# resero-labs/latok

Measured on AMD Instinct MI355X. Metric: input UTF-8 GB/s tokenized (fused feature+split-mask path), higher is better.
Workload: dtype u64

## Files before the change

### latok_amd/csrc/api.cpp

```cpp
#include <hip/hip_runtime.h>
#include <errno.h>
#include <fcntl.h>
#include <stdarg.h>
#include <stdio.h>
#include <stdlib.h>
#include <string.h>
#include <sys/mman.h>
#include <sys/stat.h>
#include <unistd.h>

#include <algorithm>
#include <array>
#include <atomic>
#include <chrono>
#include <mutex>
#include <new>
#include <string>
#include <thread>
#include <vector>

#include "../../include/latok_hip.h"
#include "corpus_gen.h"
#include "flow_hazards.h"
#include "kernels.h"
#include "unicode_tables.inc"

static_assert(LATOK_TBL_SHIFT == latok::kTblShift, "table shift");
static_assert(LATOK_TBL_STAGE1_LEN == latok::kStage1Len, "stage-1 length");
static_assert(LATOK_TBL_NBLOCKS * (1 << LATOK_TBL_SHIFT) == latok::kStage2Len, "stage-2 length");
static_assert(LATOK_TILE_CHARS == latok::kTile, "tile size");

namespace {

thread_local std::string g_err;

int fail(int code, const char* fmt, ...) {
    char buf[512];
    va_list ap;
    va_start(ap, fmt);
    vsnprintf(buf, sizeof(buf), fmt, ap);
    va_end(ap);
    g_err = buf;
    return code;
}
#define HIP_TRY(expr)                                                                                     \
    do {                                                                                                  \
        hipError_t e_ = (expr);                                                                           \
        if (e_ != hipSuccess) return fail(LATOK_ERR_HIP, "%s failed: %s", #expr, hipGetErrorString(e_)); \
    } while (0)

struct DevBuf {
    void* p = nullptr;
    size_t cap = 0;
    unsigned gen = 0;
    int ensure(size_t bytes) {
        if (bytes <= cap) return LATOK_OK;
        ++gen;
        if (p) (void)hipFree(p);
        p = nullptr;
        cap = 0;
        size_t want = bytes + bytes / 8 + 256;
        hipError_t e = hipMalloc(&p, want);
        if (e != hipSuccess) {
            p = nullptr;
            return fail(LATOK_ERR_NOMEM, "hipMalloc(%zu) failed: %s", want, hipGetErrorString(e));
        }
        cap = want;
        return LATOK_OK;
    }
    void release() {
        if (p) (void)hipFree(p);
        p = nullptr;
        cap = 0;
    }
};

struct PinBuf {
// ... 263 lines not shown
    P.u8 = in.form == Form::Utf32 ? nullptr : (const uint8_t*)in.p;
    P.row_off = a.b.row;
    P.n_str = n_str;
    P.total = total;
    P.n_tiles = n_tiles;
    const int n_cu = g.plan_cus > 0 ? g.plan_cus : g.n_cu;
    const bool one_launch_ok = a.stages == 7 && in.form == Form::Utf32 && !a.tiles_begin && !a.tiles_end && one_segment_enabled();
    latok::LaunchPlan L;
    latok::plan_launch(n_tiles, n_cu, &w != &g.ws, mode, one_launch_ok, &L);
    P.seg_tiles = L.seg_tiles;
    P.n_segs = L.n_segs;
    const bool one_launch = L.one_launch != 0;
    if ((size_t)P.n_segs * (sizeof(latok::Fn64) + sizeof(latok::Hd64)) > w.seg_agg.cap || (size_t)n_tiles * 16 > w.summ.cap)
        return fail(LATOK_ERR_INVALID, "internal: workspace too small for %lld segments / %lld tiles", (long long)P.n_segs, (long long)n_tiles);
    if (a.codes && mode != latok::kModeBits && mode != latok::kModeRules)
        return fail(LATOK_ERR_INVALID, "internal: code bytes are written by the UTF-32 bitmask modes only");
    const uint8_t* tables = (const uint8_t*)((latok::mode_rules(mode) || a.codes) ? g.t1rule.p : g.t1.p);
    P.t1 = tables;
    P.t2 = tables + latok::kStage1Pad;
    if (latok::mode_base(mode) == latok::kModeBytes) {
        P.t1 = (const uint8_t*)(latok::mode_rules(mode) ? g.tb6rule.p : g.tb6.p);
        P.t2 = P.t1 + latok::kB6Stage1Bytes;
    }
    if (latok::mode_rules(mode)) P.rules = g.rules;
    else memset(&P.rules, 0, sizeof(P.rules));
    P.bits_out = a.bits;
    P.values_out = a.values;
    P.space_out = a.space;
    P.lead_out = a.lead;
    P.lead_pref_out = a.lead_pref;
    P.lead_cnt_out = a.lead_cnt;
    P.codes_out = a.codes;
    P.tile_first = (int64_t*)w.tile_first.p;
    P.summ = (int4*)w.summ.p;
    P.seg_fn = (latok::Fn64*)w.seg_agg.p;
    P.seg_hd = (latok::Hd64*)((char*)w.seg_agg.p + (size_t)P.n_segs * sizeof(latok::Fn64));
    P.fix_count = (int64_t*)w.fix_count.p;
    P.bm_a1 = a.bm_a1;
    P.bm_a2 = a.bm_a2;
    P.bm_flags = a.bm_flags;
    P.done = (a.stages & 4) ? a.done : latok::DoneSignal{nullptr, 0, nullptr};
    g.last.plan = L;
    g.last.n_tiles = n_tiles;
    g.last.mode = mode;
    g.last.small = g.pin.d && in.p == g.pin.d;
    g.last.fix_count = (const int64_t*)w.fix_count.p;
    g.last.st = a.st;
    g.last.valid = true;
    const hipStream_t st = a.st;
    if (one_launch) {
        HIP_TRY(latok::launch_one_segment(P, mode, st));
        return LATOK_OK;
    }
    if (a.stages & 1) HIP_TRY(latok::launch_tile_index(P, st));
    if (a.tiles_begin) HIP_TRY(hipEventRecord(a.tiles_begin, st));
    if (a.stages & 2) HIP_TRY(latok::launch_split_tiles(P, mode, L, st));
    if (a.tiles_end) HIP_TRY(hipEventRecord(a.tiles_end, st));
    if (a.stages & 4) HIP_TRY(latok::launch_resolve_fix(P, mode, L, st));
    return LATOK_OK;
}

int check_csr_host(const int64_t* row_off, int64_t n_str, int64_t* total_io) {
    if (n_str < 0) return fail(LATOK_ERR_INVALID, "n_str must be >= 0");
    if (n_str == 0) { *total_io = 0; return LATOK_OK; }
    if (!row_off) return fail(LATOK_ERR_INVALID, "row_off is NULL");
    if (row_off[0] != 0) return fail(LATOK_ERR_INVALID, "row_off[0] must be 0");
    for (int64_t s = 0; s < n_str; ++s)
        if (row_off[s + 1] < row_off[s]) return fail(LATOK_ERR_INVALID, "row_off must be non-decreasing");
    if (*total_io >= 0 && *total_io != row_off[n_str])
        return fail(LATOK_ERR_INVALID, "total_chars does not match row_off[n_str]");
    *total_io = row_off[n_str];
    return LATOK_OK;
}

int resolve_total_device(const int64_t* d_row, int64_t n_str, int64_t* total_io, hipStream_t st) {
    if (n_str < 0) return fail(LATOK_ERR_INVALID, "n_str must be >= 0");
    if (n_str == 0) { *total_io = 0; return LATOK_OK; }
    if (*total_io < 0) {
        HIP_TRY(hipMemcpyAsync(total_io, d_row + n_str, 8, hipMemcpyDeviceToHost, st));
        HIP_TRY(hipStreamSynchronize(st));
    }
    return LATOK_OK;
}

int resolve_total(const int64_t* row_off, int64_t n_str, int64_t* total_io, bool dev, hipStream_t st) {
    return dev ? resolve_total_device(row_off, n_str, total_io, st) : check_csr_host(row_off, n_str, total_io);
}

int arm_done(Ctx& g, hipStream_t st, latok::DoneSignal* done) {
    *done = latok::DoneSignal{nullptr, 0, nullptr};
    if (!poll_completion()) return LATOK_OK;
    int rc;
    if ((rc = g.pin_tot.ensure(64)) || (rc = g.done_ctr.ensure(64))) return rc;
    if (g.done_ctr.gen != g.done_ctr_seen) {
        g.done_ctr_seen = g.done_ctr.gen;
        HIP_TRY(hipMemsetAsync(g.done_ctr.p, 0, 64, st));
    }
    *done = latok::DoneSignal{(unsigned long long*)g.pin_tot.d + 2, ++g.small_seq, (unsigned*)g.done_ctr.p};
    return LATOK_OK;
}
int wait_done(Ctx& g, const latok::DoneSignal& done, hipStream_t st) {
    if (!(done.word && wait_completion_word((const unsigned long long*)g.pin_tot.h + 2, done.seq))) HIP_TRY(hipStreamSynchronize(st));
    return LATOK_OK;
}

int units_on_device(Ctx& g, const Batch& b, bool dev, hipStream_t st, Batch* d) {
    *d = b;
// ... 1768 lines not shown
}
int latok_utf8_bytes(const uint32_t* cps, int64_t n, int64_t* bytes_out, int flags) {
    if (!bytes_out || n < 0) return fail(LATOK_ERR_INVALID, "bad args");
    if (!(flags & LATOK_DEVICE_PTRS)) {
        int64_t t = 0;
        for (int64_t i = 0; i < n; ++i) t += latok_utf8_len(cps[i]);
        *bytes_out = t;
        return LATOK_OK;
    }
    LATOK_ENTER();
    int rc = need_init(g);
    if (rc) return rc;
    HIP_TRY(latok::launch_utf8_bytes(cps, n, (unsigned long long*)g.ws.scalar.p, g.stream));
    unsigned long long t = 0;
    HIP_TRY(hipMemcpyAsync(&t, g.ws.scalar.p, 8, hipMemcpyDeviceToHost, g.stream));
    HIP_TRY(hipStreamSynchronize(g.stream));
    *bytes_out = (int64_t)t;
    return LATOK_OK;
}

int latok_debug_set_scan_epoch(unsigned epoch) {
    LATOK_ENTER();
    g.ws.scan_epoch = epoch & 0x3FFFFu;
    return LATOK_OK;
}

extern "C" int latok_debug_limits(int64_t* out, int n) {
    const int64_t v[17] = {latok::kTile, latok::kWPB, latok::kNarrowWPB, latok::kSegMax, latok::kOneSegTiles, latok::kFastTailTiles,
                           kSmallChars, kSmallStrings, latok::kCompressWaves, latok::kFeatWaves, latok::kFeatRound, latok::kFeatRoundTm,
                           latok::kFeatFormThresh, latok::kFeatWinBytes, latok::kHashWaveBytes, latok::scan_small_max(),
                           latok::utf8_block_bytes()};
    if (!out || n < 0) return fail(LATOK_ERR_INVALID, "NULL output");
    const int k = n < 17 ? n : 17;
    for (int i = 0; i < k; ++i) out[i] = v[i];
    return k;
}

static int put_plan(const latok::LaunchPlan& L, int64_t n_tiles, int64_t* out, int n) {
    const int64_t v[12] = {L.n_cu_eff, L.seg_tiles, L.n_segs, L.rounds, L.grid, L.one_launch ? 0 : L.grid, L.fast_tail, L.pf, L.wpb, L.nw,
                           L.one_launch, n_tiles};
    const int k = n < 12 ? n : 12;
    for (int i = 0; i < k; ++i) out[i] = v[i];
    return k;
}

extern "C" int latok_debug_plan(int64_t n_tiles, int n_cu, int in_flow, int mode, int64_t* out, int n) {
    if (!out || n < 0 || n_tiles < 1 || n_cu < 1 || mode < latok::kModeBits || mode > latok::kModeValuesRules)
        return fail(LATOK_ERR_INVALID, "n_tiles >= 1, n_cu >= 1, mode 0..%d", latok::kModeValuesRules);
    latok::LaunchPlan L;
    latok::plan_launch(n_tiles, n_cu, in_flow != 0, mode, one_segment_enabled(), &L);
    return put_plan(L, n_tiles, out, n);
}

extern "C" int latok_debug_set_plan_cus(int n_cu) {
    LATOK_ENTER();
    int rc = need_init(g);
    if (rc) return rc;
    if (n_cu != 0 && (n_cu < 8 || n_cu > g.n_cu)) return fail(LATOK_ERR_INVALID, "plan CUs must be 0 or 8..%d", g.n_cu);
    g.plan_cus = n_cu;
    return LATOK_OK;
}

extern "C" int latok_debug_last_plan(int64_t* out, int n) {
    LATOK_ENTER();
    int rc = need_init(g);
    if (rc) return rc;
    if (!out || n < 0) return fail(LATOK_ERR_INVALID, "NULL output");
    if (!g.last.valid) return 0;
    int64_t fix = 0;
    HIP_TRY(hipStreamSynchronize(g.last.st));
    HIP_TRY(hipMemcpy(&fix, g.last.fix_count, 8, hipMemcpyDeviceToHost));
    const int64_t head[3] = {g.last.mode, g.last.small ? 1 : 0, fix};
    int k = 0;
    for (; k < 3 && k < n; ++k) out[k] = head[k];
    if (n > 3) k += put_plan(g.last.plan, g.last.n_tiles, out + 3, n - 3);
    return k;
}

extern "C" int latok_debug_last_route(void) {
    LATOK_ENTER();
    return g.last_route;
}

extern "C" int latok_debug_flow_route(int n_slots, const uint64_t* lo, const uint64_t* bytes, const int* is_write, int n, int* drained_out) {
    static thread_local latok::FlowHazards held;
    static thread_local unsigned long long seq = 0;
    if (drained_out) *drained_out = 0;
    if (n < 0) { held.clear(); seq = 0; return 0; }
    if (n_slots < 1 || n_slots > latok::FlowHazards::kMaxSlots || n > 16) return fail(LATOK_ERR_INVALID, "1..4 slots, <= 16 ranges");
    latok::FlowRange r[16];
    for (int i = 0; i < n; ++i) r[i] = latok::flow_range((const void*)(uintptr_t)lo[i], (size_t)bytes[i], is_write[i] != 0);
    const int turn = (int)(seq % (unsigned)n_slots);
    int s = held.route(n_slots, turn, r, n);
    if (s == latok::FlowHazards::kDrainFirst) {
        held.clear();
        if (drained_out) *drained_out = 1;
        s = turn;
    }
    held.note(s, r, n);
    ++seq;
    return s;
}

extern "C" int latok_debug_host_decode_utf8(const uint8_t* utf8, const int64_t* byte_off, int64_t n_str, uint32_t* cps_out,
                                            int64_t* cp_row_out, int64_t* bytepos_out, int64_t* n_cps_out) {
    int64_t total = -1;
// ... 910 lines not shown
```

### latok_amd/csrc/aux_kernels.hip

```cpp
#include <hip/hip_runtime.h>
#include <stdint.h>

#include "corpus_gen.h"
#include "kernels.h"
#include "utf8_decode.h"
#include "wave_ops.h"

namespace latok {

__device__ __forceinline__ uint32_t base_word(const uint8_t* t1, const uint8_t* t2cls, const uint16_t* cw, uint32_t cp) {
    const uint32_t hi = min(cp >> kTblShift, (uint32_t)(kStage1Len - 1));
    return cw[t2cls[((uint32_t)t1[hi] << kTblShift) | (cp & ((1u << kTblShift) - 1u))]];
}

__device__ __forceinline__ uint32_t feature_row_bits(uint32_t w, uint32_t p, uint32_t x, uint32_t y, bool first, bool last) {
    uint32_t r = w & 0xFFFu;
    r |= ((p >> 0) & 1u) << 12;
    r |= ((x >> 0) & 1u) << 13;
    r |= ((p >> 1) & 1u) << 14;
    r |= ((x >> 1) & 1u) << 15;
    r |= ((p >> 3) & 1u) << 16;
    r |= ((x >> 3) & 1u) << 17;
    r |= (first ? 1u : (p >> 5) & 1u) << 18;
    r |= (last ? 1u : (x >> 5) & 1u) << 19;
    r |= ((p >> 6) & 1u) << 20;
    r |= ((x >> 8) & 1u) << 21;
    r |= ((x >> 10) & 1u) << 22;
    r |= ((y >> 0) & 1u) << 23;
    r |= ((y >> 10) & 1u) << 24;
    return r;
}

__global__ void k_parse_matrix(const uint32_t* __restrict__ cps, int64_t n, const uint8_t* __restrict__ t1,
                               const uint8_t* __restrict__ t2cls, const uint16_t* __restrict__ cw,
                               int8_t* __restrict__ out) {
    const int64_t i = (int64_t)blockIdx.x * blockDim.x + threadIdx.x;
    if (i >= n) return;
    const uint32_t w = base_word(t1, t2cls, cw, cps[i]);
    const uint32_t p = i > 0 ? base_word(t1, t2cls, cw, cps[i - 1]) : 0u;
    const uint32_t x = i + 1 < n ? base_word(t1, t2cls, cw, cps[i + 1]) : 0u;
    const uint32_t y = i + 2 < n ? base_word(t1, t2cls, cw, cps[i + 2]) : 0u;
    const uint32_t bits = feature_row_bits(w, p, x, y, i == 0, i + 1 == n);
    int8_t* row = out + i * 25;
#pragma unroll
    for (int c = 0; c < 25; ++c) row[c] = (int8_t)((bits >> c) & 1u);
}

hipError_t launch_parse_matrix(const uint32_t* cps, int64_t n, const uint8_t* t1, const uint8_t* t2cls,
                               const uint16_t* cw, int8_t* out, hipStream_t st) {
    if (n <= 0) return hipSuccess;
    const int threads = 256;
    hipLaunchKernelGGL(k_parse_matrix, dim3((unsigned)((n + threads - 1) / threads)), dim3(threads), 0, st, cps, n, t1,
                       t2cls, cw, out);
    return hipGetLastError();
}

__global__ __launch_bounds__(256) void k_parse_matrix_small(const uint32_t* __restrict__ cps, int n, const uint8_t* __restrict__ t1,
// ... 356 lines not shown
hipError_t launch_utf8_decode(const uint8_t* u8, int64_t total, const int64_t* byte_off, int64_t n_str,
                              const int64_t* block_base, uint16_t* chunk_pref, int64_t total_cps, uint32_t* cps,
                              int64_t* cp_off, hipStream_t st) {
    hipLaunchKernelGGL(k_utf8_decode_chunks, dim3((unsigned)utf8_blocks(total)), dim3(kU8Threads), 0, st, u8, total,
                       block_base, chunk_pref, cps);
    hipLaunchKernelGGL(k_utf8_cp_offsets, dim3((unsigned)((n_str + 1 + 255) / 256)), dim3(256), 0, st, u8, total, byte_off,
                       n_str, block_base, chunk_pref, total_cps, cp_off);
    return hipGetLastError();
}

template <typename T>
__global__ void k_widen_units(const T* __restrict__ units, int64_t n, uint32_t* __restrict__ cps) {
    const int64_t i0 = ((int64_t)blockIdx.x * blockDim.x + threadIdx.x) * 4;
    if (i0 + 4 <= n && ((uintptr_t)units & (4 * sizeof(T) - 1)) == 0) {
        T u[4];
        if (sizeof(T) == 1) *reinterpret_cast<uint32_t*>(u) = *reinterpret_cast<const uint32_t*>(units + i0);
        else *reinterpret_cast<uint2*>(u) = *reinterpret_cast<const uint2*>(units + i0);
        *reinterpret_cast<uint4*>(cps + i0) = make_uint4(u[0], u[1], u[2], u[3]);
    } else {
        for (int64_t i = i0; i < n && i < i0 + 4; ++i) cps[i] = units[i];
    }
}

hipError_t launch_widen_units(const void* units, int kind, int64_t n, uint32_t* cps, hipStream_t st) {
    if (n <= 0) return hipSuccess;
    const unsigned blocks = (unsigned)((n + 1023) / 1024);
    if (kind == 1) hipLaunchKernelGGL(k_widen_units<uint8_t>, dim3(blocks), dim3(256), 0, st, (const uint8_t*)units, n, cps);
    else hipLaunchKernelGGL(k_widen_units<uint16_t>, dim3(blocks), dim3(256), 0, st, (const uint16_t*)units, n, cps);
    return hipGetLastError();
}

__global__ void k_corpus_fill(uint64_t seed, int model, uint64_t sid0, int64_t n_str,
                              const int64_t* __restrict__ row_off, uint32_t* __restrict__ cps) {
    const int64_t s = (int64_t)blockIdx.x * blockDim.x + threadIdx.x;
    if (s >= n_str) return;
    const int64_t b = row_off[s];
    latok_corpus_string(seed, model, sid0 + (uint64_t)s, cps + b, row_off[s + 1] - b);
}

hipError_t launch_corpus_fill(uint64_t seed, int model, uint64_t sid0, int64_t n_str, const int64_t* row_off,
                              uint32_t* cps, hipStream_t st) {
    if (n_str <= 0) return hipSuccess;
    hipLaunchKernelGGL(k_corpus_fill, dim3((unsigned)((n_str + 63) / 64)), dim3(64), 0, st, seed, model, sid0, n_str,
                       row_off, cps);
    return hipGetLastError();
}

typedef uint32_t stream_u32x4 __attribute__((ext_vector_type(4)));
__global__ void __launch_bounds__(512) k_stream_read(const stream_u32x4* __restrict__ src, int64_t n_steps,
                                                     uint32_t* __restrict__ sink) {
    const int lane = threadIdx.x & 63;
    const int64_t wave = ((int64_t)blockIdx.x * blockDim.x + threadIdx.x) >> 6;
    const int64_t n_waves = ((int64_t)gridDim.x * blockDim.x) >> 6;
    uint32_t acc = 0;
    for (int64_t t = wave; t < n_steps; t += n_waves) {
        const stream_u32x4* p = src + t * 1024 + lane;
        stream_u32x4 v[16];
#pragma unroll
        for (int i = 0; i < 16; ++i) v[i] = __builtin_nontemporal_load(p + 64 * i);
#pragma unroll
        for (int i = 0; i < 16; ++i) acc ^= v[i].x ^ v[i].y ^ v[i].z ^ v[i].w;
    }
    if (acc == 0x9E3779B9u) sink[0] = acc;
}

hipError_t launch_stream_read(const void* src, int64_t bytes, uint32_t* sink, int n_cu, hipStream_t st) {
    const int64_t n_steps = bytes / 16384;
    if (n_steps <= 0) return hipSuccess;
    hipLaunchKernelGGL(k_stream_read, dim3((unsigned)(n_cu * 2)), dim3(512), 0, st, (const stream_u32x4*)src, n_steps, sink);
    return hipGetLastError();
}

__global__ void k_utf8_bytes(const uint32_t* __restrict__ cps, int64_t n, unsigned long long* __restrict__ total) {
    long long local = 0;
    for (int64_t i = (int64_t)blockIdx.x * blockDim.x + threadIdx.x; i < n; i += (int64_t)gridDim.x * blockDim.x)
        local += latok_utf8_len(cps[i]);
#pragma unroll
    for (int d = 32; d >= 1; d >>= 1) local += __shfl_xor(local, d);
    if ((threadIdx.x & 63) == 0) atomicAdd(total, (unsigned long long)local);
}

hipError_t launch_utf8_bytes(const uint32_t* cps, int64_t n, unsigned long long* total, hipStream_t st) {
    hipError_t e = hipMemsetAsync(total, 0, sizeof(unsigned long long), st);
    if (e != hipSuccess || n <= 0) return e;
    int64_t blocks = (n + 255) / 256;
    if (blocks > 4096) blocks = 4096;
    hipLaunchKernelGGL(k_utf8_bytes, dim3((unsigned)blocks), dim3(256), 0, st, cps, n, total);
    return hipGetLastError();
}

}
```

### latok_amd/csrc/kernels.h

```cpp
#ifndef LATOK_KERNELS_H
#define LATOK_KERNELS_H
#include <hip/hip_runtime.h>
#include <stdint.h>

#include "split_code.h"

namespace latok {

constexpr int kTile = 4096;
constexpr int kTblShift = 7;
constexpr int kStage1Len = 8705;
constexpr int kStage1Pad = 8720;
constexpr int kStage2Len = 255 * 128;
constexpr int kTablesLdsBytes = kStage1Pad + kStage2Len;
constexpr int kB6Stage1Len = LK_B6_STAGE1_LEN;
constexpr int kB6Stage1Bytes = (kB6Stage1Len * 2 + 1023) / 1024 * 1024;
constexpr int kB6MaxBlocks = 400;
constexpr int kB6Stage2Bytes = kB6MaxBlocks * 64;
constexpr int kB6TablesBytes = kB6Stage1Bytes + kB6Stage2Bytes;
static_assert(kB6Stage1Bytes % 1024 == 0 && kB6Stage2Bytes % 1024 == 0 && kB6Stage1Bytes <= kTablesLdsBytes, "byte space keeps its stage 1 where the other modes keep both stages");
constexpr int kStageBytes = 64 * 80;
constexpr int kWaveLdsBytes = kStageBytes + 16 + 65 * 8 + 8;

constexpr int kModeBits = 0;
constexpr int kModeValues = 1;
constexpr int kModeBlockMask = 2;
constexpr int kModeRules = 3;
constexpr int kModeBytes = 4;
constexpr int kModeLatin1 = 5;
constexpr int kModeUcs2 = 6;
constexpr int kModeBytesRules = 7;
constexpr int kModeLatin1Rules = 8;
constexpr int kModeUcs2Rules = 9;
constexpr int kModeValuesRules = 10;
constexpr int mode_base(int mode) {
    return mode == kModeRules ? kModeBits : mode == kModeBytesRules ? kModeBytes : mode == kModeLatin1Rules ? kModeLatin1
         : mode == kModeUcs2Rules ? kModeUcs2 : mode == kModeValuesRules ? kModeValues : mode;
}
constexpr bool mode_rules(int mode) { return mode != mode_base(mode); }
constexpr int mode_with_rules(int base) {
    return base == kModeBits ? kModeRules : base == kModeBytes ? kModeBytesRules : base == kModeLatin1 ? kModeLatin1Rules
         : base == kModeUcs2 ? kModeUcs2Rules : base == kModeValues ? kModeValuesRules : base;
}
constexpr bool mode_is_bytes(int mode) { return mode_base(mode) == kModeBytes || mode_base(mode) == kModeLatin1 || mode_base(mode) == kModeUcs2; }
constexpr bool mode_is_units(int mode) { return mode_base(mode) == kModeLatin1 || mode_base(mode) == kModeUcs2; }
constexpr bool mode_writes_bits(int mode) { return mode_base(mode) == kModeBits || mode_is_bytes(mode); }

constexpr long long kNegInf64 = -(1ll << 60);
constexpr int kWPB = 12;
constexpr int kSegMax = kWPB * 64;

struct Fn64 {
    long long a, b;
};
struct Hd64 {
    long long h;
    int c;
};

struct DoneSignal {
    unsigned long long* word;
    unsigned long long seq;
    unsigned* counter;
};
#if defined(__HIPCC__)
__device__ __forceinline__ void signal_block_done(const DoneSignal& d) {
    if (!d.word) return;
    __threadfence_system();
    __syncthreads();
    if (threadIdx.x == 0) {
        const unsigned n = gridDim.x;
        if (__hip_atomic_fetch_add(d.counter, 1u, __ATOMIC_ACQ_REL, __HIP_MEMORY_SCOPE_AGENT) == n - 1u) {
            *d.counter = 0u;
            __threadfence_system();
            __hip_atomic_store(d.word, d.seq, __ATOMIC_RELEASE, __HIP_MEMORY_SCOPE_SYSTEM);
        }
    }
}
#endif

struct SplitParams {
    const uint32_t* cps;
    const uint8_t* u8;
    const int64_t* row_off;
    int64_t n_str, total, n_tiles;
    int seg_tiles;
    int64_t n_segs;
    const uint8_t* t1;
    const uint8_t* t2;
    uint64_t* bits_out;
    uint8_t* values_out;
    uint64_t* space_out;
    uint64_t* lead_out;
    uint16_t* lead_pref_out;
    int64_t* lead_cnt_out;
    uint8_t* codes_out;
    int64_t* tile_first;
    int4* summ;
    Fn64* seg_fn;
// ... 139 lines not shown
```

### latok_amd/csrc/split_kernels.hip

```cpp
#include <hip/hip_runtime.h>
#include <stdint.h>
#include <stdlib.h>

#include "bitscan.h"
#include "feat_records.h"
#include "kernels.h"
#include "tile_core.h"

namespace latok {

#ifdef LATOK_STAMPS
__device__ unsigned long long g_stamp_sum[16];
__device__ unsigned long long g_stamp_cnt;
#endif

__device__ __forceinline__ Fn64 fn_then(Fn64 f1, Fn64 f2) {
    Fn64 f;
    const bool c1 = f1.a <= kNegInf64, c2 = f2.a <= kNegInf64;
    if (c2) { f.a = kNegInf64; f.b = f2.b; return f; }
    f.a = c1 ? kNegInf64 : f1.a + f2.a;
    const long long c = f1.b + f2.a;
    f.b = c > f2.b ? c : f2.b;
    return f;
}
__device__ __forceinline__ long long fn_apply(Fn64 f, long long q) {
    if (f.a <= kNegInf64) return f.b;
    const long long c = q + f.a;
    return c > f.b ? c : f.b;
}
__device__ __forceinline__ Fn64 fn_of(int4 s) {
    Fn64 f;
    f.a = s.x <= LK_NEG_INF / 2 ? kNegInf64 : (long long)s.x;
    f.b = s.y;
    return f;
}
__device__ __forceinline__ Hd64 hd_then(Hd64 x, Hd64 y) {
    Hd64 r;
    r.c = x.c | y.c;
    r.h = x.c ? x.h : x.h + y.h;
    return r;
}

constexpr int kScanWaves = kWPB;

__device__ __forceinline__ Fn64 fn_identity() { Fn64 f; f.a = 0; f.b = 0; return f; }
__device__ __forceinline__ Hd64 hd_identity() { Hd64 h; h.h = 0; h.c = 0; return h; }

template <int NW>
struct ScanLdsT {
    Fn64 fn_w[NW];
    Hd64 hd_w[NW];
};
typedef ScanLdsT<kScanWaves> ScanLds;
template <int NW = kScanWaves>
__device__ __forceinline__ void block_scan(Fn64 f, Hd64 h, ScanLdsT<NW>& L, Fn64* excl_fn, Hd64* excl_hd, Fn64* tot_fn,
                                           Hd64* tot_hd) {
    const int lane = threadIdx.x & 63, wave = threadIdx.x >> 6;
    Fn64 fi = f;
    Hd64 hi = h;
#pragma unroll
// ... 147 lines not shown
    }
}
__device__ __attribute__((noinline, cold)) void tables_fetch_bytes(const uint8_t* t1, const uint8_t* t2, uint8_t* tables, int* ctl) {
    const int lane = (int)(threadIdx.x & 63u);
    struct { const uint8_t* t1; const uint8_t* t2; } P = {t1, t2};
    struct { uint8_t* tables; int* ctl; } L = {tables, ctl};
    typedef const void __attribute__((address_space(1))) * gptr_t;
    typedef void __attribute__((address_space(3))) * lptr_t;
    for (;;) {
        const int ticket = __hip_atomic_fetch_add(&L.ctl[0], 1, __ATOMIC_RELAXED, __HIP_MEMORY_SCOPE_WORKGROUP);
        const int g = __builtin_amdgcn_readfirstlane(ticket) >> 6;
        if (g >= kLazyGrabs) break;
        if (g == kLazyGrabs - 1) {
#pragma unroll
            for (int j = 0; j < 4; ++j) {
                const lk_lead_entry e = lk_lead_entry_of((uint32_t)(64 * j + lane));
                reinterpret_cast<uint2*>(L.tables + kLdsLeadTab)[64 * j + lane] = make_uint2(e.sel, e.hi0);
            }
        } else {
#pragma unroll
            for (int j = 0; j < kLazyPer; ++j) {
                const int row = g * kLazyPer + j;
                if (row < kLazyRows)
                    __builtin_amdgcn_global_load_lds((gptr_t)(P.t1 + 1024 * row + 16 * lane), (lptr_t)(L.tables + 1024 * row), 16, 0, 0);
            }
            __builtin_amdgcn_s_waitcnt(0x0F70);
        }
        __hip_atomic_fetch_add(&L.ctl[1], 1, __ATOMIC_RELEASE, __HIP_MEMORY_SCOPE_WORKGROUP);
    }
    while (__hip_atomic_load(&L.ctl[1], __ATOMIC_ACQUIRE, __HIP_MEMORY_SCOPE_WORKGROUP) < 64 * kLazyGrabs) __builtin_amdgcn_s_sleep(2);
}

template <int MODE = kModeBits>
__device__ __forceinline__ TileLds wave_lds(uint8_t* lds, int wave) {
    TileLds L;
    L.t1 = lds;
    L.t2 = lds + kStage1Pad;
    uint8_t* const w = lds + lds_shift(MODE);
    uint8_t* mine = wave < kWPB ? w + kLdsWaves + wave * kWaveLdsBytes : lds + lds_total(MODE) + (wave - kWPB) * kWaveLdsBytes;
    L.stage = mine;
    L.halo = mine + kStageBytes;
    L.bw = reinterpret_cast<lk_u64*>(mine + kStageBytes + 16);
    L.lut = lds;
    L.ltab = lds + kLdsLeadTab;
    L.tables = lds;
    L.ctl = reinterpret_cast<int*>(w + kLdsMisc) + 16;
    L.t1b = lds;
    L.t2b = lds + kB6Stage1Bytes;
    L.ctab = mode_base(MODE) == kModeBytes ? lds + kLdsByteCodes : L.lut + kSliceLutBytes;
    L.small_bits = L.small_space = nullptr;
    return L;
}

template <int MODE, bool FAST_TAIL = false, int WPB = kWPB, int PF = kCpsPrefetchRows>
__device__ __forceinline__ void run_segment(const SplitParams& P, uint8_t* lds, int64_t seg, int tid, int lane,
                                            int wave, bool tables LATOK_STAMP_PARAM) {
    const int S = P.seg_tiles;
    const TileLds L = wave_lds<MODE>(lds, wave);
    int4* sm = reinterpret_cast<int4*>(lds + lds_shift(MODE) + kLdsSumm);
    ScanLdsT<WPB>& scan = *reinterpret_cast<ScanLdsT<WPB>*>(lds + lds_shift(MODE) + kLdsScan);

    const int64_t T0 = seg * S;
    const int64_t T1 = min(T0 + S, P.n_tiles);
    const int n_seg = (int)(T1 - T0);
    int64_t tfv = 0;
    if (wave + WPB * lane < n_seg) tfv = P.tile_first[T0 + wave + WPB * lane];
    tfv = tfv < 0 ? 0 : (tfv > P.n_str ? P.n_str : tfv);
    if (tables) __syncthreads();
    constexpr bool kDefer = mode_writes_bits(MODE) && !mode_is_bytes(MODE);
    lk_u64 obuf[8];
    int slot = 0, k_first = wave;
    const int64_t n_words = (P.total + 63) >> 6;
    auto flush = [&]() {
#pragma unroll
        for (int j = 0; j < 8; ++j) {
            if (j < slot) {
                const int64_t w = (T0 + k_first + j * WPB) * 64 + lane;
                if (w < n_words) P.bits_out[w] = obuf[j];
            }
        }
        slot = 0;
    };
    auto put = [&](lk_u64 w, int k) {
        if (slot == 0) k_first = k;
#pragma unroll
        for (int j = 0; j < 8; ++j) obuf[j] = (j == slot) ? w : obuf[j];
        if (++slot == 8) flush();
    };
    CpsPrefetch pf;
    pf.valid = false;
    for (int k = wave, j = 0; k < n_seg; k += WPB, ++j) {
        const lk_u64 w = process_tile<MODE, kDefer, false, FAST_TAIL, PF>(P, L, T0 + k, lane_read64(tfv, j), 0, -1, true, &sm[k], lane LATOK_STAMP_ARG
                                                                      , MODE == kModeBits && !FAST_TAIL ? &pf : nullptr, k + WPB < n_seg ? T0 + k + WPB : (int64_t)-1
                                                                      );
        if (kDefer) put(w, k);
#ifdef LATOK_STAMPS
        stamp_acc[0] += 1;
#endif
    }
    if (kDefer) flush();
    __syncthreads();
    {
        Fn64 f = fn_identity();
        Hd64 h = hd_identity();
        if (tid < n_seg) {
            const int4 s = sm[tid];
            P.summ[T0 + tid] = s;
            f = fn_of(s);
            h.h = s.z; h.c = s.w & 1;
        }
        Fn64 ef, tfn; Hd64 eh, th;
        block_scan<WPB>(f, h, scan, &ef, &eh, &tfn, &th);
        if (tid == 0) { P.seg_fn[seg] = tfn; P.seg_hd[seg] = th; }
    }
    __syncthreads();
}

template <int MODE, bool FAST_TAIL = false, int PF = kCpsPrefetchRows>
__global__ __launch_bounds__(tile_wpb(MODE) * 64) void k_tiles_main(SplitParams P) {
    constexpr int WPB = tile_wpb(MODE);
    __shared__ __attribute__((aligned(16))) uint8_t lds[lds_total_tiles(MODE)];
    const int tid = threadIdx.x;
    const int lane = tid & 63;
    const int wave = __builtin_amdgcn_readfirstlane(tid >> 6);
    if (blockIdx.x == 0 && tid == 0) *P.fix_count = 0;

    bool tables = MODE != kModeBlockMask;
    if (tables) {
        if (mode_base(MODE) == kModeBytes) load_tables_ascii_bytes(lds, P);
        else load_tables<WPB * 64, MODE>(lds, P);
    }
#ifdef LATOK_STAMPS
    unsigned long long stamp_acc[16];
    for (int i = 0; i < 16; ++i) stamp_acc[i] = 0;
#endif
    for (int64_t seg = blockIdx.x; seg < P.n_segs; seg += gridDim.x) {
        run_segment<MODE, FAST_TAIL, WPB, PF>(P, lds, seg, tid, lane, wave, tables LATOK_STAMP_ARG);
        tables = false;
    }
#ifdef LATOK_STAMPS
    if (lane == 0)
        for (int i = 0; i < 16; ++i) atomicAdd(&g_stamp_sum[i], stamp_acc[i]);
#endif
}

template <int MODE, int NW, bool ONE>
__device__ __forceinline__ void resolve_segments(const SplitParams& P, uint8_t* lds, int tid, int lane, int wave) {
    const int S = P.seg_tiles;
    ScanLdsT<NW>& scan = *reinterpret_cast<ScanLdsT<NW>*>(lds + lds_shift(MODE) + kLdsScan);
    int* misc = reinterpret_cast<int*>(lds + lds_shift(MODE) + kLdsMisc);
    int* fix_t = reinterpret_cast<int*>(lds + lds_shift(MODE) + kLdsTf);
    int2* fix_in = reinterpret_cast<int2*>(lds + lds_shift(MODE) + kLdsSumm);
    bool tables_loaded = ONE;

    for (int64_t seg = ONE ? 0 : (int64_t)blockIdx.x; seg < (ONE ? 1 : P.n_segs); seg += ONE ? 1 : (int64_t)gridDim.x) {
        const int64_t T0 = seg * S;
        const int64_t T1 = min(T0 + S, P.n_tiles);
        const int n_seg = (int)(T1 - T0);
        if (tid == 0) misc[0] = 0;
        const int64_t t = T0 + tid;
        int4 s = make_int4(0, 0, 0, 0);
        if (tid < n_seg) s = P.summ[t];
        Fn64 pf = fn_identity();
        Hd64 sh = hd_identity();
        if (P.n_segs > 1) {
            const int64_t per = (P.n_segs + NW * 64 - 1) / (NW * 64);
            const int64_t lo = min((int64_t)tid * per, P.n_segs), hi = min(lo + per, P.n_segs);
            Fn64 f = fn_identity();
            Hd64 h = hd_identity();
            for (int64_t j = lo; j < hi; ++j) {
                if (j < seg) f = fn_then(f, P.seg_fn[j]);
                if (j > seg) h = hd_then(h, P.seg_hd[j]);
            }
            Fn64 ef; Hd64 eh;
            block_scan<NW>(f, h, scan, &ef, &eh, &pf, &sh);
        }
        const long long q_seg_in = fn_apply(pf, 0);
        Hd64 rest; rest.h = sh.h; rest.c = 1;

        Fn64 f = fn_identity();
        Hd64 h = hd_identity();
        if (tid < n_seg) {
            f = fn_of(s);
            h.h = s.z; h.c = s.w & 1;
        }
        Fn64 ef, tfn; Hd64 eh, th;
        block_scan<NW>(f, h, scan, &ef, &eh, &tfn, &th);
        if (tid < n_seg) {
            const long long q_in = fn_apply(ef, q_seg_in);
            const long long q_end = fn_apply(f, q_in);
            const long long h_next = hd_then(eh, rest).h;
// ... 46 lines not shown
                process_tile<MODE>(P, L, tt, idx0, in.x, in.y, false, nullptr, lane);
            }
            if (tid == 0) atomicAdd(reinterpret_cast<unsigned long long*>(P.fix_count), (unsigned long long)n_fix);
        }
        __syncthreads();
    }
}

template <int MODE, int NW>
__global__ __launch_bounds__(NW * 64) void k_resolve_fix(SplitParams P) {
    __shared__ __attribute__((aligned(16))) uint8_t lds[lds_total(MODE)];
    const int tid = threadIdx.x;
    const int lane = tid & 63;
    const int wave = __builtin_amdgcn_readfirstlane(tid >> 6);
    resolve_segments<MODE, NW, false>(P, lds, tid, lane, wave);
    signal_block_done(P.done);
}

__device__ __forceinline__ void tile_index_entry(const int64_t* __restrict__ row_off, int64_t n_str, int64_t n_tiles,
                                                 int64_t* __restrict__ tile_first, int64_t s, int lane) {
    int64_t w0 = 0, w1 = -1;
    if (s <= n_str) {
        const int64_t p = row_off[s];
        const int64_t prev = s > 0 ? row_off[s - 1] : -1;
        w0 = prev < 0 ? 0 : prev / kTile + 1;
        w1 = p / kTile;
        if (w1 > n_tiles - 1) w1 = n_tiles - 1;
    }
    const bool wide = w1 - w0 >= 16;
    if (!wide)
        for (int64_t w = w0; w <= w1; ++w) tile_first[w] = s;
    unsigned long long m = __ballot(wide);
    while (m) {
        const int src = __ffsll((long long)m) - 1;
        m &= m - 1;
        const int64_t a = lane_read64(w0, src), b = lane_read64(w1, src), v = lane_read64(s, src);
        for (int64_t w = a + lane; w <= b; w += 64) tile_first[w] = v;
    }
}


template <int MODE>
__global__ __launch_bounds__(kWPB * 64) void k_one_segment(SplitParams P) {
    __shared__ __attribute__((aligned(16))) uint8_t lds[lds_total(MODE)];
    const int tid = threadIdx.x;
    const int lane = tid & 63;
    const int wave = __builtin_amdgcn_readfirstlane(tid >> 6);
    if (tid == 0) *P.fix_count = 0;
    load_tables<kWPB * 64, MODE>(lds, P);
    for (int64_t base = 0; base <= P.n_str; base += kWPB * 64)
        tile_index_entry(P.row_off, P.n_str, P.n_tiles, P.tile_first, base + tid, lane);
    __threadfence_block();
    __syncthreads();
    run_segment<MODE, true>(P, lds, 0, tid, lane, wave, true LATOK_STAMP_NULL);
    __threadfence_block();
    __syncthreads();
    resolve_segments<MODE, kWPB, true>(P, lds, tid, lane, wave);
    signal_block_done(P.done);
}

__global__ void k_any_nonzero(const int8_t* __restrict__ a1, const int8_t* __restrict__ a2, int64_t n,
                              int* __restrict__ flags) {
    int f1 = 0, f2 = 0;
    for (int64_t i = (int64_t)blockIdx.x * blockDim.x + threadIdx.x; i < n; i += (int64_t)gridDim.x * blockDim.x) {
        f1 |= a1[i] != 0;
        f2 |= a2[i] != 0;
    }
    if (__any(f1) && (threadIdx.x & 63) == 0) atomicOr(&flags[0], 1);
    if (__any(f2) && (threadIdx.x & 63) == 0) atomicOr(&flags[1], 1);
}

hipError_t launch_any_nonzero(const int8_t* a1, const int8_t* a2, int64_t n, int* flags, hipStream_t st) {
    hipError_t e = hipMemsetAsync(flags, 0, 2 * sizeof(int), st);
    if (e != hipSuccess || n <= 0) return e;
    int64_t blocks = (n + 255) / 256;
    if (blocks > 1024) blocks = 1024;
    hipLaunchKernelGGL(k_any_nonzero, dim3((unsigned)blocks), dim3(256), 0, st, a1, a2, n, flags);
    return hipGetLastError();
}

struct SmallParams {
    SplitParams P;
    void* counts;
    void* items;
    int64_t* n_items;
    unsigned long long* done;
    unsigned long long seq;
    int8_t* features;
};

template <int MODE, int KIND, typename OUT>
__global__ __launch_bounds__(64) void k_small_batch(SmallParams S) {
    __shared__ __attribute__((aligned(16))) uint8_t lds[kWaveLdsBytes];
    __shared__ uint64_t s_bits[66], s_space[66], s_items[66];
    __shared__ int s_pref[66];
    const int lane = threadIdx.x;
    TileLds L;
    L.t1 = S.P.t1;
    L.t2 = S.P.t2;
    L.lut = L.ctab = L.ltab = L.t1b = L.t2b = nullptr; L.tables = nullptr; L.ctl = nullptr;
    L.stage = lds;
    L.halo = lds + kStageBytes;
    L.bw = reinterpret_cast<lk_u64*>(lds + kStageBytes + 16);
    s_bits[lane] = 0ull;
    s_space[lane] = ~0ull;
    if (lane < 2) { s_bits[64 + lane] = 0ull; s_space[64 + lane] = ~0ull; }
    const SplitParams& P = S.P;
// ... 337 lines not shown
```

### latok_amd/csrc/tile_core.h

```cpp
#ifndef LATOK_TILE_CORE_H
#define LATOK_TILE_CORE_H
#include <hip/hip_runtime.h>
#include <stdint.h>

#include "kernels.h"
#include "lane_math.h"
#include "utf8_decode.h"
#include "wave_ops.h"

namespace latok {

#ifdef LATOK_STAMPS
#define LATOK_STAMP(k)                                                                           \
    do {                                                                                         \
        __builtin_amdgcn_sched_barrier(0);                                                       \
        unsigned long long t_;                                                                   \
        asm volatile("s_memtime %0\n\ts_waitcnt lgkmcnt(0)" : "=s"(t_)::"memory");            \
        __builtin_amdgcn_sched_barrier(0);                                                       \
        if ((k) > 0) stamp_acc[(k)] += t_ - stamp_prev;                                          \
        stamp_prev = t_;                                                                         \
    } while (0)
#define LATOK_STAMP_ARG , stamp_acc
#define LATOK_STAMP_PARAM , unsigned long long* stamp_acc
#define LATOK_STAMP_NULL , nullptr
// ... 681 lines not shown
                            for (int c = 0; c < LK_COUNT_BITS; ++c) {
                                v |= (int)((counts.split[c] >> i) & 1) << c;
                                vy |= (int)((counts.sym[c] >> i) & 1) << c;
                            }
                        } else {
                            v = (int)((loc.t_space >> i) & 1) + (int)((loc.t_sym >> i) & 1) + (int)((loc.t_prevsym >> i) & 1) +
                                (int)((loc.t_camel_next >> i) & 1) + (int)((loc.t_camel_prev >> i) & 1);
                            vy = (int)((loc.sym >> i) & 1);
                        }
                        v = ((keep >> i) & 1) ? v : 0;
                        v += vy;
                        if ((B >> i) & 1) v = 1;
                        packed |= (uint32_t)v << (8 * b);
                    }
                }
                if (4 * w + 4 <= n) {
                    *reinterpret_cast<uint32_t*>(dst + 4 * w) = packed;
                } else {
                    for (int b = 0; b < 4 && 4 * w + b < n; ++b) dst[4 * w + b] = (uint8_t)(packed >> (8 * b));
                }
            }
        }
    }
    if (mode_base(MODE) == kModeBytes && !SMALL && P.lead_out) {
        const int64_t remain = total - base;
        const lk_u64 valid = remain >= 64 ? ~0ull : (remain <= 0 ? 0ull : ((1ull << remain) - 1ull));
        const lk_u64 leadw = ~cont_plane & valid;
        const int cnt = lk_popc(leadw);
        int inc = cnt;
        inc += dpp_mov<kDppRowShr1, 0xF>(0, inc);
        inc += dpp_mov<kDppRowShr2, 0xF>(0, inc);
        inc += dpp_mov<kDppRowShr4, 0xF>(0, inc);
        inc += dpp_mov<kDppRowShr8, 0xF>(0, inc);
        inc += dpp_mov<kDppRowBcast15, 0xA>(0, inc);
        inc += dpp_mov<kDppRowBcast31, 0xC>(0, inc);
        if (base < total) {
            P.lead_out[base >> 6] = leadw;
            P.lead_pref_out[base >> 6] = (uint16_t)(inc - cnt);
        }
        if (lane == 63) P.lead_cnt_out[t] = inc;
    }
    LATOK_STAMP(8);
    wave_lds_sync();
    return out_word;
}


template <int MODE, bool DEFER = false, bool SMALL = false, bool FAST_TAIL = false, int PF = kCpsPrefetchRows>
__device__ __forceinline__ lk_u64 process_tile(const SplitParams& P, const TileLds& L, int64_t t, int64_t idx0, int q_in,
                                             int tail_zero, bool write_summary, int4* summ_l, int lane
#ifdef LATOK_STAMPS
                                             , unsigned long long* stamp_acc = nullptr
#endif
                                             , CpsPrefetch* pf = nullptr, int64_t t_next = -1
                                             ) {
#ifdef LATOK_STAMPS
    unsigned long long stamp_prev = 0, stamp_dummy[16];
    if (!stamp_acc) stamp_acc = stamp_dummy;
#endif
    const int64_t t0 = t * kTile;
    const int64_t total = P.total;
    const uint32_t st_lane = 4u * lane + 16u * ((uint32_t)lane >> 4);
    bool raw_stage = mode_base(MODE) == kModeLatin1;
    bool ascii_tile = false;
    bool tile_not_ascii = false;
    LATOK_STAMP(0);

    int64_t ro = idx0 + lane <= P.n_str ? P.row_off[idx0 + lane] : INT64_MAX;
    uint32_t halo_cp = 0xFFFFFFFFu;
    if (MODE != kModeBlockMask && !mode_is_bytes(MODE) && lane < 3) {
        const int64_t hp = lane == 0 ? t0 - 1 : t0 + kTile + (lane - 1);
        if (hp >= 0 && hp < total) halo_cp = P.cps[hp];
    }

    if (MODE == kModeBlockMask) {
    } else if (mode_base(MODE) == kModeLatin1) {
        ascii_tile = units_phase1<1>(P, L, t0, lane);
    } else if (mode_base(MODE) == kModeUcs2) {
        units_phase1<2>(P, L, t0, lane);
    } else if (mode_base(MODE) == kModeBytes) {
        raw_stage = bytes_phase1(P, L, t0, lane
#ifdef LATOK_STAMPS
                                 , stamp_acc, stamp_prev
#endif
                                 );
        ascii_tile = raw_stage;
    } else if (FAST_TAIL) {
        const bool full = t0 + kTile <= total;
        u32x4 v[16];
        const u32x4* src = reinterpret_cast<const u32x4*>(P.cps + t0) + lane;
        const int64_t remain0 = total - t0 - 4 * (int64_t)lane;
        int n_rows = 16;
        if (full) {
#pragma unroll
            for (int i = 0; i < 16; ++i) v[i] = __builtin_nontemporal_load(src + 64 * i);
        } else {
            const int64_t last_blk = (total - 1) & ~(int64_t)3;
            n_rows = (int)((total - t0 + 255) >> 8);
#pragma unroll
            for (int i = 0; i < 16; ++i) {
                if (i < n_rows) {
                    int64_t p = t0 + 256 * i + 4 * (int64_t)lane;
                    p = p < last_blk ? p : last_blk;
                    v[i] = __builtin_nontemporal_load(reinterpret_cast<const u32x4*>(P.cps + p));
                }
            }
        }
        uint32_t* codes = P.codes_out ? reinterpret_cast<uint32_t*>(P.codes_out + t0) + lane : nullptr;
#pragma unroll
        for (int i = 0; i < 16; ++i) {
            uint32_t c = 0;
            if (i < n_rows) {
                c = classify4(L.t1, L.t2, v[i]);
                if (!full) {
                    const int64_t remain = remain0 - 256 * i;
                    c &= remain >= 4 ? 0xFFFFFFFFu : (remain <= 0 ? 0u : ((1u << (8 * (int)remain)) - 1u));
                }
            }
            *reinterpret_cast<uint32_t*>(L.stage + st_lane + 320u * i) = c;
            if (codes) codes[64 * i] = c;
        }
    } else if (t0 + kTile <= total) {
        u32x4 v[16];
        const u32x4* src = reinterpret_cast<const u32x4*>(P.cps + t0) + lane;
        constexpr int R = PF;
        const bool pre = R > 0 && pf && pf->valid;
#pragma unroll
        for (int i = 0; i < 16; ++i) {
            if (i < R && pre) v[i] = pf->v[i < R ? i : 0];
            else v[i] = __builtin_nontemporal_load(src + 64 * i);
        }
        LATOK_STAMP(1);
        uint32_t* codes = P.codes_out ? reinterpret_cast<uint32_t*>(P.codes_out + t0) + lane : nullptr;
#pragma unroll
        for (int i = 0; i < 16; ++i) {
            const uint32_t c = classify4(L.t1, L.t2, v[i], &tile_not_ascii);
            *reinterpret_cast<uint32_t*>(L.stage + st_lane + 320u * i) = c;
            if (codes) codes[64 * i] = c;
        }
    } else {
        uint32_t* codes = P.codes_out ? reinterpret_cast<uint32_t*>(P.codes_out + t0) + lane : nullptr;
#pragma unroll 1
        for (int i = 0; i < 16; ++i) {
            const int64_t p = t0 + 256 * i + 4 * lane;
            u32x4 v;
            v.x = p + 0 < total ? P.cps[p + 0] : 0xFFFFFFFFu;
            v.y = p + 1 < total ? P.cps[p + 1] : 0xFFFFFFFFu;
            v.z = p + 2 < total ? P.cps[p + 2] : 0xFFFFFFFFu;
            v.w = p + 3 < total ? P.cps[p + 3] : 0xFFFFFFFFu;
            const uint32_t c = classify4(L.t1, L.t2, v);
            *reinterpret_cast<uint32_t*>(L.stage + st_lane + 320u * i) = c;
            if (codes) codes[64 * i] = c;
        }
    }
    if (MODE != kModeBlockMask && !mode_is_bytes(MODE) && lane < 3) L.halo[lane] = (uint8_t)classify1(L.t1, L.t2, halo_cp);
    L.bw[lane] = 0;
    if (lane == 0) L.bw[64] = 0;
    LATOK_STAMP(2);
    wave_lds_sync();
    for (;;) {
        const int64_t rel = ro - t0;
        if (rel >= 0 && rel < kTile + 64) atomicOr(&L.bw[rel >> 6], 1ull << (rel & 63));
        const int64_t last = lane_read64(ro, 63);
        if (last >= t0 + kTile + 64) break;
        idx0 += 64;
        ro = idx0 + lane <= P.n_str ? P.row_off[idx0 + lane] : INT64_MAX;
    }
    wave_lds_sync();
    LATOK_STAMP(3);
    if (MODE == kModeBits && pf) {
        __builtin_amdgcn_s_waitcnt(0x0F70);
        pf->valid = false;
        const bool want = true;
        if (want && t_next >= 0 && (t_next + 1) * kTile <= total) {
            const u32x4* nsrc = reinterpret_cast<const u32x4*>(P.cps + t_next * kTile) + lane;
#pragma unroll
            for (int i = 0; i < PF; ++i) pf->v[i] = __builtin_nontemporal_load(nsrc + 64 * i);
            pf->valid = true;
        }
    }

    return tile_phase2<MODE, DEFER, SMALL>(P, L, t, q_in, tail_zero, write_summary, summ_l, lane, raw_stage, ascii_tile
#ifdef LATOK_STAMPS
                                    , stamp_acc, stamp_prev
#endif
                                    );
}

}
#endif
```

Before: 1492.

## Assign contiguous tile runs per wave and derive tile-first indices inline

For bits/rules modes, each wave now processes a contiguous run of tiles in a segment instead of strided tiles. It locates the first string index of its run with an interpolation probe over row_off plus a wave-level search, then carries the next tile's first index forward out of the boundary-scan loop. This removes the separate tile_index kernel launch and its global round trip, and the probe load is issued before the table load to overlap latency. Tile_first is still written out for later stages. The stream-read benchmark kernel also switches to contiguous runs. Risks are load imbalance when tile costs vary and mispredicted probes falling back to a full lower-bound search.

```diff
diff --git a/latok_amd/csrc/api.cpp b/latok_amd/csrc/api.cpp
--- a/latok_amd/csrc/api.cpp
+++ b/latok_amd/csrc/api.cpp
@@ -23,6 +23,7 @@
 #include "corpus_gen.h"
 #include "flow_hazards.h"
 #include "kernels.h"
+#include "tile_runs.h"
 #include "unicode_tables.inc"
 
 static_assert(LATOK_TBL_SHIFT == latok::kTblShift, "table shift");
@@ -392,7 +393,8 @@
         HIP_TRY(latok::launch_one_segment(P, mode, st));
         return LATOK_OK;
     }
-    if (a.stages & 1) HIP_TRY(latok::launch_tile_index(P, st));
+    const bool index_launch = (a.stages & 1) && !(latok::mode_owns_runs(mode) && (a.stages & 2));
+    if (index_launch) HIP_TRY(latok::launch_tile_index(P, st));
     if (a.tiles_begin) HIP_TRY(hipEventRecord(a.tiles_begin, st));
     if (a.stages & 2) HIP_TRY(latok::launch_split_tiles(P, mode, L, st));
     if (a.tiles_end) HIP_TRY(hipEventRecord(a.tiles_end, st));
@@ -2267,6 +2269,12 @@
     return put_plan(L, n_tiles, out, n);
 }
 
+extern "C" int latok_debug_tile_run(int n_seg, int wpb, int wave, int* start, int* len) {
+    if (!start || !len || n_seg < 0 || wpb < 1 || wave < 0) return fail(LATOK_ERR_INVALID, "n_seg >= 0, wpb >= 1, wave >= 0, outputs not NULL");
+    lk_tile_run<int>(n_seg, wpb, wave, start, len);
+    return LATOK_OK;
+}
+
 extern "C" int latok_debug_set_plan_cus(int n_cu) {
     LATOK_ENTER();
     int rc = need_init(g);
diff --git a/latok_amd/csrc/aux_kernels.hip b/latok_amd/csrc/aux_kernels.hip
--- a/latok_amd/csrc/aux_kernels.hip
+++ b/latok_amd/csrc/aux_kernels.hip
@@ -3,6 +3,7 @@
 
 #include "corpus_gen.h"
 #include "kernels.h"
+#include "tile_runs.h"
 #include "utf8_decode.h"
 #include "wave_ops.h"
 
@@ -465,8 +466,10 @@
     const int lane = threadIdx.x & 63;
     const int64_t wave = ((int64_t)blockIdx.x * blockDim.x + threadIdx.x) >> 6;
     const int64_t n_waves = ((int64_t)gridDim.x * blockDim.x) >> 6;
+    int64_t t0, len;
+    lk_tile_run<int64_t>(n_steps, n_waves, wave, &t0, &len);
     uint32_t acc = 0;
-    for (int64_t t = wave; t < n_steps; t += n_waves) {
+    for (int64_t t = t0; t < t0 + len; ++t) {
         const stream_u32x4* p = src + t * 1024 + lane;
         stream_u32x4 v[16];
 #pragma unroll
diff --git a/latok_amd/csrc/kernels.h b/latok_amd/csrc/kernels.h
--- a/latok_amd/csrc/kernels.h
+++ b/latok_amd/csrc/kernels.h
@@ -45,6 +45,7 @@
 constexpr bool mode_is_bytes(int mode) { return mode_base(mode) == kModeBytes || mode_base(mode) == kModeLatin1 || mode_base(mode) == kModeUcs2; }
 constexpr bool mode_is_units(int mode) { return mode_base(mode) == kModeLatin1 || mode_base(mode) == kModeUcs2; }
 constexpr bool mode_writes_bits(int mode) { return mode_base(mode) == kModeBits || mode_is_bytes(mode); }
+constexpr bool mode_owns_runs(int mode) { return mode == kModeBits || mode == kModeRules; }
 
 constexpr long long kNegInf64 = -(1ll << 60);
 constexpr int kWPB = 12;
diff --git a/latok_amd/csrc/split_kernels.hip b/latok_amd/csrc/split_kernels.hip
--- a/latok_amd/csrc/split_kernels.hip
+++ b/latok_amd/csrc/split_kernels.hip
@@ -6,6 +6,7 @@
 #include "feat_records.h"
 #include "kernels.h"
 #include "tile_core.h"
+#include "tile_runs.h"
 
 namespace latok {
 
@@ -259,9 +260,47 @@
     return L;
 }
 
-template <int MODE, bool FAST_TAIL = false, int WPB = kWPB, int PF = kCpsPrefetchRows>
+constexpr int kProbeStride = 32;
+struct RunProbe {
+    int64_t c;
+    int64_t base;
+    int64_t v;
+};
+__device__ __forceinline__ RunProbe run_probe_place(const SplitParams& P, int64_t t) {
+    RunProbe r;
+    r.c = t * kTile;
+    const int64_t centre = (int64_t)((double)P.n_str * ((double)r.c / (double)P.total));
+    const int64_t base = centre - 32 * kProbeStride;
+    r.base = base < 0 ? 0 : base;
+    r.v = 0;
+    return r;
+}
+__device__ __forceinline__ int64_t run_probe_load(const SplitParams& P, const RunProbe& r, int lane) {
+    const int64_t p = r.base + (int64_t)kProbeStride * lane;
+    return p <= P.n_str ? P.row_off[p] : INT64_MAX;
+}
+__device__ __forceinline__ int64_t run_probe_finish(const SplitParams& P, const RunProbe& r, int lane) {
+    int64_t ans = -1;
+    const uint64_t m = __ballot(r.v >= r.c);
+    if (m) {
+        const int f = __builtin_ctzll(m);
+        if (f == 0) {
+            if (r.base == 0) ans = 0;
+        } else {
+            const int64_t q0 = r.base + (int64_t)kProbeStride * (f - 1) + 1;
+            const int64_t q = q0 + lane;
+            const int64_t v = q <= P.n_str ? P.row_off[q] : INT64_MAX;
+            const uint64_t m2 = __ballot(v >= r.c);
+            if (m2) ans = q0 + __builtin_ctzll(m2);
+        }
+    }
+    if (ans < 0) ans = wave_lower_bound(P.row_off, P.n_str + 1, r.c, lane);
+    return to_scalar64(ans > P.n_str ? P.n_str : ans);
+}
+
+template <int MODE, bool FAST_TAIL = false, int WPB = kWPB, int PF = kCpsPrefetchRows, bool RUNS = mode_owns_runs(MODE)>
 __device__ __forceinline__ void run_segment(const SplitParams& P, uint8_t* lds, int64_t seg, int tid, int lane,
-                                            int wave, bool tables LATOK_STAMP_PARAM) {
+                                            int wave, bool tables, bool have_early, int64_t early_v LATOK_STAMP_PARAM) {
     const int S = P.seg_tiles;
     const TileLds L = wave_lds<MODE>(lds, wave);
     int4* sm = reinterpret_cast<int4*>(lds + lds_shift(MODE) + kLdsSumm);
@@ -271,18 +310,31 @@
     const int64_t T1 = min(T0 + S, P.n_tiles);
     const int n_seg = (int)(T1 - T0);
     int64_t tfv = 0;
-    if (wave + WPB * lane < n_seg) tfv = P.tile_first[T0 + wave + WPB * lane];
-    tfv = tfv < 0 ? 0 : (tfv > P.n_str ? P.n_str : tfv);
+    int r_start = 0, r_len = 0;
+    int64_t idx_run = 0;
+    if (RUNS) {
+        lk_tile_run<int>(n_seg, WPB, wave, &r_start, &r_len);
+        if (r_len > 0) {
+            RunProbe pr = run_probe_place(P, T0 + r_start);
+            pr.v = have_early ? early_v : run_probe_load(P, pr, lane);
+            idx_run = run_probe_finish(P, pr, lane);
+        }
+    } else {
+        if (wave + WPB * lane < n_seg) tfv = P.tile_first[T0 + wave + WPB * lane];
+        tfv = tfv < 0 ? 0 : (tfv > P.n_str ? P.n_str : tfv);
+    }
     if (tables) __syncthreads();
     constexpr bool kDefer = mode_writes_bits(MODE) && !mode_is_bytes(MODE);
+    constexpr int kStep = RUNS ? 1 : WPB;
+    const int k_begin = RUNS ? r_start : wave, k_end = RUNS ? r_start + r_len : n_seg;
     lk_u64 obuf[8];
-    int slot = 0, k_first = wave;
+    int slot = 0, k_first = k_begin;
     const int64_t n_words = (P.total + 63) >> 6;
     auto flush = [&]() {
 #pragma unroll
         for (int j = 0; j < 8; ++j) {
             if (j < slot) {
-                const int64_t w = (T0 + k_first + j * WPB) * 64 + lane;
+                const int64_t w = (T0 + k_first + j * kStep) * 64 + lane;
                 if (w < n_words) P.bits_out[w] = obuf[j];
             }
         }
@@ -296,16 +348,20 @@
     };
     CpsPrefetch pf;
     pf.valid = false;
-    for (int k = wave, j = 0; k < n_seg; k += WPB, ++j) {
-        const lk_u64 w = process_tile<MODE, kDefer, false, FAST_TAIL, PF>(P, L, T0 + k, lane_read64(tfv, j), 0, -1, true, &sm[k], lane LATOK_STAMP_ARG
-                                                                      , MODE == kModeBits && !FAST_TAIL ? &pf : nullptr, k + WPB < n_seg ? T0 + k + WPB : (int64_t)-1
-                                                                      );
+    int64_t tf_out = 0;
+    for (int k = k_begin, j = 0; k < k_end; k += kStep, ++j) {
+        const int64_t idx0 = RUNS ? idx_run : lane_read64(tfv, j);
+        if (RUNS && lane == j) tf_out = idx0;
+        const lk_u64 w = process_tile<MODE, kDefer, false, FAST_TAIL, PF>(P, L, T0 + k, idx0, 0, -1, true, &sm[k], lane LATOK_STAMP_ARG
+                                                                      , MODE == kModeBits && !FAST_TAIL ? &pf : nullptr, k + kStep < k_end ? T0 + k + kStep : (int64_t)-1
+                                                                      , RUNS ? &idx_run : nullptr);
         if (kDefer) put(w, k);
 #ifdef LATOK_STAMPS
         stamp_acc[0] += 1;
 #endif
     }
     if (kDefer) flush();
+    if (RUNS && P.tile_first && lane < r_len) P.tile_first[T0 + r_start + lane] = tf_out;
     __syncthreads();
     {
         Fn64 f = fn_identity();
@@ -333,6 +389,17 @@
     if (blockIdx.x == 0 && tid == 0) *P.fix_count = 0;
 
     bool tables = MODE != kModeBlockMask;
+    int64_t probe_v = 0;
+    bool probed = false;
+    if (mode_owns_runs(MODE) && (int64_t)blockIdx.x < P.n_segs) {
+        const int64_t T0 = (int64_t)blockIdx.x * P.seg_tiles;
+        int r_start, r_len;
+        lk_tile_run<int>((int)(min(T0 + P.seg_tiles, P.n_tiles) - T0), WPB, wave, &r_start, &r_len);
+        if (r_len > 0) {
+            probe_v = run_probe_load(P, run_probe_place(P, T0 + r_start), lane);
+            probed = true;
+        }
+    }
     if (tables) {
         if (mode_base(MODE) == kModeBytes) load_tables_ascii_bytes(lds, P);
         else load_tables<WPB * 64, MODE>(lds, P);
@@ -342,8 +409,9 @@
     for (int i = 0; i < 16; ++i) stamp_acc[i] = 0;
 #endif
     for (int64_t seg = blockIdx.x; seg < P.n_segs; seg += gridDim.x) {
-        run_segment<MODE, FAST_TAIL, WPB, PF>(P, lds, seg, tid, lane, wave, tables LATOK_STAMP_ARG);
+        run_segment<MODE, FAST_TAIL, WPB, PF>(P, lds, seg, tid, lane, wave, tables, probed, probe_v LATOK_STAMP_ARG);
         tables = false;
+        probed = false;
     }
 #ifdef LATOK_STAMPS
     if (lane == 0)
@@ -496,7 +564,7 @@
         tile_index_entry(P.row_off, P.n_str, P.n_tiles, P.tile_first, base + tid, lane);
     __threadfence_block();
     __syncthreads();
-    run_segment<MODE, true>(P, lds, 0, tid, lane, wave, true LATOK_STAMP_NULL);
+    run_segment<MODE, true, kWPB, kCpsPrefetchRows, false>(P, lds, 0, tid, lane, wave, true, false, 0 LATOK_STAMP_NULL);
     __threadfence_block();
     __syncthreads();
     resolve_segments<MODE, kWPB, true>(P, lds, tid, lane, wave);
diff --git a/latok_amd/csrc/tile_core.h b/latok_amd/csrc/tile_core.h
--- a/latok_amd/csrc/tile_core.h
+++ b/latok_amd/csrc/tile_core.h
@@ -757,7 +757,7 @@
 #ifdef LATOK_STAMPS
                                              , unsigned long long* stamp_acc = nullptr
 #endif
-                                             , CpsPrefetch* pf = nullptr, int64_t t_next = -1
+                                             , CpsPrefetch* pf = nullptr, int64_t t_next = -1, int64_t* next_first = nullptr
                                              ) {
 #ifdef LATOK_STAMPS
     unsigned long long stamp_prev = 0, stamp_dummy[16];
@@ -863,14 +863,24 @@
     if (lane == 0) L.bw[64] = 0;
     LATOK_STAMP(2);
     wave_lds_sync();
+    int64_t nf = idx0;
+    bool nf_found = false;
     for (;;) {
         const int64_t rel = ro - t0;
         if (rel >= 0 && rel < kTile + 64) atomicOr(&L.bw[rel >> 6], 1ull << (rel & 63));
+        if (next_first && !nf_found) {
+            const lk_u64 ge = __ballot(ro >= t0 + kTile);
+            if (ge) {
+                nf = idx0 + lk_ctz(ge);
+                nf_found = true;
+            }
+        }
         const int64_t last = lane_read64(ro, 63);
         if (last >= t0 + kTile + 64) break;
         idx0 += 64;
         ro = idx0 + lane <= P.n_str ? P.row_off[idx0 + lane] : INT64_MAX;
     }
+    if (next_first) *next_first = nf > P.n_str ? P.n_str : nf;
     wave_lds_sync();
     LATOK_STAMP(3);
     if (MODE == kModeBits && pf) {
diff --git a/latok_amd/csrc/tile_runs.h b/latok_amd/csrc/tile_runs.h
--- /dev/null
+++ b/latok_amd/csrc/tile_runs.h
@@ -0,0 +1,24 @@
+#ifndef LATOK_TILE_RUNS_H
+#define LATOK_TILE_RUNS_H
+#include <stdint.h>
+
+#if defined(__HIPCC__)
+#include <hip/hip_runtime.h>
+#define LK_RUN_FN __host__ __device__ inline
+#else
+#define LK_RUN_FN inline
+#endif
+
+template <typename T>
+LK_RUN_FN void lk_tile_run(T n, T wpb, T wave, T* start, T* len) {
+    if (n <= 0 || wpb <= 0 || wave < 0 || wave >= wpb) {
+        *start = n > 0 ? n : 0;
+        *len = 0;
+        return;
+    }
+    const T base = n / wpb, rem = n % wpb;
+    *start = wave * base + (wave < rem ? wave : rem);
+    *len = base + (wave < rem ? 1 : 0);
+}
+
+#endif
```

Result: slower. 1476 (-1.0%).
